# Nikhil-AI-Labs/image-super-resolution-2

Measured on AMD Instinct MI355X. Metric: output MPix/s at x4 SR (256->1024), higher is better.
Workload: dtype bf16 (bf16 MFMA operands, fp32 accumulate, fp32 activations in HBM); 1 GPU; FreqFusion x4 full 3-expert forward (HAT-L + DAT + NAFNet-SR + fusion stack), one 256x256 LR tile -> 1024x1024 per step per GPU (BASELINE configs[1]); seeded synthetic weights (172.3 M params), 1/f-noise tiles; tile=256, parallelism=tile-sharded x1, weights RCCL-broadcast once (0.0 ms), no per-tile collectives, launch=hipGraph replay, tiles_in_flight=2

## Files before the change

image-super-resolution-2_amd/csrc/token_linear.hip:

```cpp
#include "ff_common.h"


struct TokenLinParams {
  const float* x; float* out;
  const float* gamma; const float* beta;
  const __bf16* w;
  const float* bias;
  const float* res; const float* res2; const float* rs2;
  float* xn; int ldxn;
  float* stats; int st_lo, st_hi; float st_eps;
  const float* x2; int ldx2; const float* cm; const float* gw1t; const float* gb1; const float* gw2; float gb2;
  long long M;
  int ldx, ldo, ldr, ldr2, K, N, NT, act;
  float eps;
  int wpi;
};

#define TL_TR 36

#ifndef TL_GELU_SIG
#define TL_GELU_SIG 1
#endif
#define TL_KERNEL token_linear_kernel
#define TL_IMAGES 0
#define TL_OUT16 0
#include "token_linear_kernel.inc"
#undef TL_KERNEL
#undef TL_IMAGES
#define TL_KERNEL token_linear_images_kernel
#define TL_IMAGES 1
#include "token_linear_kernel.inc"
#undef TL_KERNEL
#undef TL_IMAGES
#undef TL_OUT16
#define TL_KERNEL token_linear_rows16_kernel
#define TL_IMAGES 0
#define TL_OUT16 1
#include "token_linear_kernel.inc"
#undef TL_KERNEL
#undef TL_IMAGES
#undef TL_OUT16


extern "C" int ff_token_linear(const float* x, int ldx, float* out, int ldo, long long M, int K, int kpad, int N, int n_tiles,
                               const float* gamma, const float* beta, float eps, const void* w_tiles,
                               const float* bias_padded, int act, const float* res, int ldr, const float* res2, int ldr2,
                               const float* res2_scale, float* xn_out, int ldxn, float* stats_out, int stat_lo, int stat_hi,
                               float stat_eps, int nterms, void* stream) {
  FF_CHECK_ARG(nterms == 1 || nterms == 3, "ff_token_linear: nterms must be 1 (plain bf16) or 3 (split bf16)");
  FF_CHECK_ARG(x && out && w_tiles, "ff_token_linear: null pointer");
  FF_CHECK_ARG(M > 0 && K > 0 && K <= 192 && K % 4 == 0 && N > 0 && n_tiles * 32 >= N, "ff_token_linear: needs K <= 192 (K %% 4 == 0), n_tiles*32 >= N");
  FF_CHECK_ARG(kpad == 64 || kpad == 128 || kpad == 192, "ff_token_linear: kpad must be 64, 128 or 192");
  FF_CHECK_ARG(kpad >= K, "ff_token_linear: kpad < K");
  FF_CHECK_ARG(ldx >= K && ldx % 4 == 0 && ldo >= N && (((uintptr_t)x) & 15) == 0, "ff_token_linear: x rows must be 16-byte aligned");
  FF_CHECK_ARG((gamma == nullptr) == (beta == nullptr), "ff_token_linear: gamma/beta come together");
  FF_CHECK_ARG((((uintptr_t)w_tiles) & 15) == 0 && (!gamma || ((((uintptr_t)gamma) & 15) == 0 && (((uintptr_t)beta) & 15) == 0)), "ff_token_linear: weights / gamma / beta must be 16-byte aligned");
  FF_CHECK_ARG(!res || ldr >= N, "ff_token_linear: ldr too small");
  FF_CHECK_ARG(!res2 || (ldr2 >= N && res2_scale), "ff_token_linear: res2 needs ldr2 >= N and a scale vector");
  FF_CHECK_ARG(!xn_out || (gamma && ldxn >= K && ldxn % 4 == 0 && (((uintptr_t)xn_out) & 15) == 0), "ff_token_linear: xn_out needs LayerNorm parameters and 16-byte aligned rows");
  TokenLinParams p;
  p.x = x; p.out = out; p.gamma = gamma; p.beta = beta; p.w = (const __bf16*)w_tiles; p.bias = bias_padded;
  p.res = res; p.res2 = res2; p.rs2 = res2_scale; p.xn = xn_out; p.ldxn = ldxn; p.M = M; p.ldx = ldx; p.ldo = ldo; p.ldr = ldr; p.ldr2 = ldr2;
  p.K = K; p.N = N; p.NT = n_tiles; p.act = act; p.eps = eps;
  FF_CHECK_ARG(!stats_out || (stat_lo >= 0 && stat_hi > stat_lo && stat_hi <= N && (((uintptr_t)stats_out) & 7) == 0), "ff_token_linear: bad statistics range");
  p.stats = stats_out; p.st_lo = stat_lo; p.st_hi = stat_hi; p.st_eps = stat_eps;
  p.x2 = nullptr; p.ldx2 = 0; p.cm = nullptr; p.gw1t = nullptr; p.gb1 = nullptr; p.gw2 = nullptr; p.gb2 = 0.f; p.wpi = 0;
  const bool vec4 = (N % 4 == 0) && (ldo % 4 == 0) && ((((uintptr_t)out) & 15) == 0) && (!res || (ldr % 4 == 0 && (((uintptr_t)res) & 15) == 0)) &&
           (!res2 || (ldr2 % 4 == 0 && (((uintptr_t)res2) & 15) == 0 && (((uintptr_t)res2_scale) & 15) == 0));
  const int ks = kpad / 16;
  const size_t lds = (size_t)2 * 2 * 32 * (2 * ks + 1) * 16 + (size_t)8 * 32 * TL_TR * 4 + (size_t)8 * 32 * FF_XS_ROW * 4 + (size_t)n_tiles * 32 * 4;
  FF_CHECK_ARG(lds <= 160 * 1024, "ff_token_linear: N too large for the LDS image");
  FF_CHECK_ARG(act == ACT_NONE || act == ACT_GELU, "ff_token_linear: act must be none or gelu");
  const long long nblk = (M + 255) / 256;
  FF_CHECK_ARG(nblk < (1LL << 31), "ff_token_linear: grid too large");
#define TL_LAUNCH(A, KSV, V4, NTM)                                                                                          \
  do {                                                                                                                      \
    static ff_device_once once;                                                                                             \
    if (!ff_raise_lds(once, "ff_token_linear", 160 * 1024, FF_LDS_SAY_ERR, &token_linear_kernel<A, KSV, V4, false, NTM>)) return FF_ERR_LAUNCH; \
    hipLaunchKernelGGL((token_linear_kernel<A, KSV, V4, false, NTM>), dim3((unsigned)nblk), dim3(512), lds, (hipStream_t)stream, p); \
  } while (0)
#define TL_LAUNCH_NT(A, KSV, V4) do { if (nterms == 3) TL_LAUNCH(A, KSV, V4, 3); else TL_LAUNCH(A, KSV, V4, 1); } while (0)
#define TL_LAUNCH_KS(A, V4) do { if (ks == 4) TL_LAUNCH_NT(A, 4, V4); else if (ks == 8) TL_LAUNCH_NT(A, 8, V4); else TL_LAUNCH_NT(A, 12, V4); } while (0)
  if (act == ACT_GELU) { if (vec4) TL_LAUNCH_KS(ACT_GELU, true); else TL_LAUNCH_KS(ACT_GELU, false); }
  else { if (vec4) TL_LAUNCH_KS(ACT_NONE, true); else TL_LAUNCH_KS(ACT_NONE, false); }
#undef TL_LAUNCH_KS
#undef TL_LAUNCH_NT
#undef TL_LAUNCH
  FF_LAUNCH_CHECK("ff_token_linear");
  return FF_OK;
}

extern "C" int ff_token_linear_rows16(const float* x, int ldx, void* out16, int ldo, long long M, int K, int kpad, int N, int n_tiles,
                                      const float* gamma, const float* beta, float eps, const void* w_tiles, const float* bias_padded,
                                      const float* col_scale, int act, const float* res, int ldr, const float* res2, int ldr2,
                                      const float* res2_scale, float* xn_out, int ldxn, float* stats_out, int stat_lo, int stat_hi,
                                      float stat_eps, int nterms, void* stream) {
  FF_CHECK_ARG(nterms == 1 && act == ACT_NONE && !res && !res2 && !res2_scale && !xn_out && !stats_out,
               "ff_token_linear_rows16: plain bf16 (nterms == 1), no activation, no res / res2 / xn_out / stats_out (got nterms=%d act=%d)", nterms, act);
  FF_CHECK_ARG(x && out16 && w_tiles && col_scale, "ff_token_linear_rows16: null pointer");
  FF_CHECK_ARG(M > 0 && K > 0 && K <= 192 && K % 4 == 0 && N > 0 && N % 4 == 0 && n_tiles * 32 >= N, "ff_token_linear_rows16: needs K <= 192, K and N multiples of 4, n_tiles*32 >= N");
  FF_CHECK_ARG(kpad == 64 || kpad == 128 || kpad == 192, "ff_token_linear_rows16: kpad must be 64, 128 or 192");
  FF_CHECK_ARG(kpad >= K, "ff_token_linear_rows16: kpad < K");
  FF_CHECK_ARG(ldx >= K && ldx % 4 == 0 && (((uintptr_t)x) & 15) == 0, "ff_token_linear_rows16: x rows must be 16-byte aligned");
  FF_CHECK_ARG(ldo >= N && ldo % 4 == 0 && (((uintptr_t)out16) & 7) == 0, "ff_token_linear_rows16: out rows must be 8-byte aligned (pitch in bf16 elements, a multiple of 4)");
  FF_CHECK_ARG((gamma == nullptr) == (beta == nullptr), "ff_token_linear_rows16: gamma/beta come together");
  FF_CHECK_ARG(((((uintptr_t)w_tiles) | ((uintptr_t)col_scale)) & 15) == 0 && (!gamma || ((((uintptr_t)gamma) & 15) == 0 && (((uintptr_t)beta) & 15) == 0)), "ff_token_linear_rows16: weights / col_scale / gamma / beta must be 16-byte aligned");
  TokenLinParams p;
  p.x = x; p.out = reinterpret_cast<float*>(out16); p.gamma = gamma; p.beta = beta; p.w = (const __bf16*)w_tiles; p.bias = bias_padded;
  p.res = nullptr; p.res2 = nullptr; p.rs2 = col_scale; p.xn = nullptr; p.ldxn = 0; p.M = M; p.ldx = ldx; p.ldo = ldo; p.ldr = 0; p.ldr2 = 0;
  p.K = K; p.N = N; p.NT = n_tiles; p.act = ACT_NONE; p.eps = eps;
  p.stats = nullptr; p.st_lo = 0; p.st_hi = 0; p.st_eps = 0.f;
  p.x2 = nullptr; p.ldx2 = 0; p.cm = nullptr; p.gw1t = nullptr; p.gb1 = nullptr; p.gw2 = nullptr; p.gb2 = 0.f; p.wpi = 0;
  const int ks = kpad / 16;
  const size_t lds = (size_t)2 * 2 * 32 * (2 * ks + 1) * 16 + (size_t)8 * 32 * TL_TR * 4 + (size_t)8 * 32 * FF_XS_ROW * 4 + (size_t)2 * n_tiles * 32 * 4;
  FF_CHECK_ARG(lds <= 160 * 1024, "ff_token_linear_rows16: N too large for the LDS image");
  const long long nblk = (M + 255) / 256;
  FF_CHECK_ARG(nblk < (1LL << 31), "ff_token_linear_rows16: grid too large");
#define TL_LAUNCH16(KSV)                                                                                                    \
  do {                                                                                                                      \
    static ff_device_once once;                                                                                             \
    if (!ff_raise_lds(once, "ff_token_linear_rows16", 160 * 1024, FF_LDS_SAY_ERR, &token_linear_rows16_kernel<ACT_NONE, KSV, true, false, 1>)) return FF_ERR_LAUNCH; \
    hipLaunchKernelGGL((token_linear_rows16_kernel<ACT_NONE, KSV, true, false, 1>), dim3((unsigned)nblk), dim3(512), lds, (hipStream_t)stream, p); \
  } while (0)
  if (ks == 4) TL_LAUNCH16(4); else if (ks == 8) TL_LAUNCH16(8); else TL_LAUNCH16(12);
#undef TL_LAUNCH16
  FF_LAUNCH_CHECK("ff_token_linear_rows16");
  return FF_OK;
}

static int token_linear_gated_launch(const char* who, const float* x, int ldx, const float* x2, int ldx2, const float* cm, int B, long long rows_per_image,
                                     const float* gw1t, const float* gb1, const float* gw2, float gb2, float* out, int ldo, long long M, int K, int N,
                                     int n_tiles, const void* w_tiles, const float* bias_padded, const float* res, int ldr, int nterms, void* stream) {
  FF_CHECK_ARG(nterms == 1 || nterms == 3, "%s: nterms must be 1 or 3", who);
  FF_CHECK_ARG(x && x2 && cm && gb1 && gw2 && out && w_tiles, "%s: null pointer", who);
  FF_CHECK_ARG(M > 0 && K > 0 && K <= 192 && K % 4 == 0 && N > 0 && N % 4 == 0 && n_tiles * 32 >= N, "%s: needs K <= 192, K and N multiples of 4", who);
  FF_CHECK_ARG(ldx >= K && ldx % 4 == 0 && ldx2 >= K && ldx2 % 4 == 0 && ldo >= N && ldo % 4 == 0 && (!res || (ldr >= N && ldr % 4 == 0)), "%s: rows must be 16-byte aligned", who);
  FF_CHECK_ARG(((((uintptr_t)x) | ((uintptr_t)x2) | ((uintptr_t)cm) | ((uintptr_t)out) | ((uintptr_t)w_tiles) | ((uintptr_t)res)) & 15) == 0, "%s: 16-byte alignment", who);
  const long long wpi = B ? rows_per_image / 256 : 0, nblk = B ? wpi : (M + 255) / 256;
  FF_CHECK_ARG(nblk < (1LL << 31), "%s: grid too large", who);
  TokenLinParams p{};
  p.x = x; p.out = out; p.w = (const __bf16*)w_tiles; p.bias = bias_padded; p.res = res; p.M = M; p.ldx = ldx; p.ldo = ldo; p.ldr = ldr;
  p.K = K; p.N = N; p.NT = n_tiles; p.act = ACT_NONE;
  p.x2 = x2; p.ldx2 = ldx2; p.cm = cm; p.gw1t = gw1t; p.gb1 = gb1; p.gw2 = gw2; p.gb2 = gb2; p.wpi = (int)wpi;
  const size_t lds = (size_t)2 * 2 * 32 * 25 * 16 + (size_t)8 * 32 * TL_TR * 4 + (size_t)8 * 32 * FF_XS_ROW * 4 + (size_t)n_tiles * 32 * 4;
  FF_CHECK_ARG(lds <= 160 * 1024, "%s: N too large for the LDS image", who);
  static ff_device_once once[2];
  if (!(!B ? ff_raise_lds(once[0], who, 160 * 1024, FF_LDS_SAY_ERR, &token_linear_kernel<ACT_NONE, 12, true, true, 3>, &token_linear_kernel<ACT_NONE, 12, true, true, 1>)
           : ff_raise_lds(once[1], who, 160 * 1024, FF_LDS_SAY_ERR, &token_linear_images_kernel<ACT_NONE, 12, true, true, 3>, &token_linear_images_kernel<ACT_NONE, 12, true, true, 1>)))
    return FF_ERR_LAUNCH;
  const dim3 grid((unsigned)nblk, B ? (unsigned)B : 1u);
  if (!B) {
    if (nterms == 3) hipLaunchKernelGGL((token_linear_kernel<ACT_NONE, 12, true, true, 3>), grid, dim3(512), lds, (hipStream_t)stream, p);
    else hipLaunchKernelGGL((token_linear_kernel<ACT_NONE, 12, true, true, 1>), grid, dim3(512), lds, (hipStream_t)stream, p);
  } else {
    if (nterms == 3) hipLaunchKernelGGL((token_linear_images_kernel<ACT_NONE, 12, true, true, 3>), grid, dim3(512), lds, (hipStream_t)stream, p);
    else hipLaunchKernelGGL((token_linear_images_kernel<ACT_NONE, 12, true, true, 1>), grid, dim3(512), lds, (hipStream_t)stream, p);
  }
  FF_LAUNCH_CHECK(who);
  return FF_OK;
}

extern "C" int ff_token_linear_gated(const float* x, int ldx, const float* x2, int ldx2, const float* cm, const float* gw1t,
                                     const float* gb1, const float* gw2, float gb2, float* out, int ldo, long long M, int K, int N,
                                     int n_tiles, const void* w_tiles, const float* bias_padded, const float* res, int ldr, int nterms,
                                     void* stream) {
  return token_linear_gated_launch("ff_token_linear_gated", x, ldx, x2, ldx2, cm, 0, 0, gw1t, gb1, gw2, gb2, out, ldo, M, K, N, n_tiles, w_tiles, bias_padded, res, ldr, nterms, stream);
}

extern "C" int ff_token_linear_gated_images(const float* x, int ldx, const float* x2, int ldx2, const float* cm, int B, long long rows_per_image,
                                            const float* gb1, const float* gw2, float gb2, float* out, int ldo, long long M, int K, int N,
                                            int n_tiles, const void* w_tiles, const float* bias_padded, const float* res, int ldr, int nterms,
                                            void* stream) {
  FF_CHECK_ARG(B > 0 && B <= 65535 && rows_per_image > 0 && rows_per_image % 256 == 0 && M == (long long)B * rows_per_image,
               "ff_token_linear_gated_images: rows_per_image must be a positive multiple of 256 and M == B * rows_per_image (1 <= B <= 65535; got B=%d rows_per_image=%lld M=%lld)",
               B, rows_per_image, M);
  return token_linear_gated_launch("ff_token_linear_gated_images", x, ldx, x2, ldx2, cm, B, rows_per_image, nullptr, gb1, gw2, gb2, out, ldo, M, K, N, n_tiles, w_tiles, bias_padded, res, ldr, nterms, stream);
}
```

image-super-resolution-2_amd/csrc/token_linear_kernel.inc:

```
template <int ACT, int TL_KS, bool VEC4, bool GATED = false, int NTERMS = 3>
__global__ __launch_bounds__(512) void TL_KERNEL(TokenLinParams p) {
  constexpr int TL_SLOTS = 2 * TL_KS + 1, TL_ROWB = TL_SLOTS * 16, TL_PL = 32 * TL_SLOTS, TL_PIECES = 2 * TL_PL / 64;
  constexpr int TL_TILE_ELEMS = 32 * 16 * TL_KS, KPAD = 16 * TL_KS;
  extern __shared__ __attribute__((aligned(16))) unsigned char smem[];
  constexpr int WB = TL_PL * 16;
  constexpr int BUFB = 2 * WB;
  const int tid = threadIdx.x, lane = tid & 63, wid = tid >> 6;
  const int l31 = lane & 31, hh = lane >> 5;
  float* tr = reinterpret_cast<float*>(smem + 2 * BUFB) + wid * (32 * TL_TR);
  float* xs = reinterpret_cast<float*>(smem + 2 * BUFB + 8 * 32 * TL_TR * 4) + wid * (32 * FF_XS_ROW);
  float* Bs = reinterpret_cast<float*>(smem + 2 * BUFB + 8 * 32 * TL_TR * 4 + 8 * 32 * FF_XS_ROW * 4);
#if TL_IMAGES
  const long long tok0 = ((long long)blockIdx.y * p.wpi + blockIdx.x) * 256 + wid * 32;
  const float* cmrow = p.cm + (long long)blockIdx.y * p.K;
#else
  const long long tok0 = (long long)blockIdx.x * 256 + wid * 32;
  const float* cmrow = p.cm;
#endif
  const long long tok = tok0 + l31;
  const bool tvalid = tok < p.M;

  int off[4];
#pragma unroll
  for (int i = 0; i < 4; ++i) {
    int s = (wid + 8 * i) * 64 + lane;
    if (s >= 2 * TL_PL) s = 2 * TL_PL - 1;
    const int plane = s / TL_PL, t = s - plane * TL_PL, row = t / TL_SLOTS;
    int q = t - row * TL_SLOTS;
    if (q > 2 * TL_KS - 1) q = 2 * TL_KS - 1;
    off[i] = plane * TL_TILE_ELEMS + row * KPAD + q * 8;
  }
  auto dma = [&](int nt, int buf) {
    const __bf16* rec = p.w + (long long)nt * (2 * TL_TILE_ELEMS);
#pragma unroll
    for (int i = 0; i < 4; ++i)
      if (wid + 8 * i < TL_PIECES)
        __builtin_amdgcn_global_load_lds((const __attribute__((address_space(1))) void*)(rec + off[i]),
                                         (__attribute__((address_space(3))) void*)(smem + buf * BUFB + (wid + 8 * i) * 1024), 16, 0, 0);
  };
  dma(0, 0);
  for (int i = tid; i < p.NT * 32; i += 512) Bs[i] = p.bias ? p.bias[i] : 0.f;
#if TL_OUT16
  float* Ss = Bs + p.NT * 32;
  for (int i = tid; i < p.NT * 32; i += 512) Ss[i] = p.rs2[i];
#endif

  bf16x8 xh[TL_KS], xl[TL_KS];
  if constexpr (GATED) {
    dma(p.NT, 1);
    float sm;
    {
      bf16x8 th[TL_KS], tl[TL_KS];
      {
        float v[TL_KS][8];
        ff_wave_rows_to_frags<TL_KS / 4>(p.x, p.ldx, tok0, p.M, p.K, xs, lane, v);
#pragma unroll
        for (int st = 0; st < TL_KS; ++st)
#pragma unroll
          for (int j = 0; j < 8; ++j) {
            const __bf16 h = (__bf16)v[st][j];
            th[st][j] = h;
            if (NTERMS == 3) tl[st][j] = (__bf16)(v[st][j] - (float)h);
          }
      }
      asm volatile("s_waitcnt vmcnt(0)" ::: "memory");
      __syncthreads();
      const unsigned char* ap = smem + BUFB + l31 * TL_ROWB + 16 * hh;
      f32x16 ga;
#pragma unroll
      for (int r = 0; r < 16; ++r) ga[r] = p.gb1[(r & 3) + 8 * (r >> 2) + 4 * hh];
#define TL_XH th
#define TL_XL tl
#define TL_ACC ga
#include "token_linear_tile_mfma.inc"
#undef TL_XH
#undef TL_XL
#undef TL_ACC
      float sacc = 0.f;
#pragma unroll
      for (int r = 0; r < 16; ++r) sacc += p.gw2[(r & 3) + 8 * (r >> 2) + 4 * hh] * ff_gelu_fast(ga[r]);
      sacc += __shfl_xor(sacc, 32);
      sm = 1.0f / (1.0f + expf(-(sacc + p.gb2)));
    }
    asm volatile("" ::: "memory");
    const int rr = lane >> 4, cq = (lane & 15) * 4;
#pragma unroll
    for (int pass = 0; pass < TL_KS / 4; ++pass) {
      asm volatile("" ::: "memory");
      f32x4 tS[8], tO[8];
#pragma unroll
      for (int j = 0; j < 8; ++j) {
        const int r = 4 * j + rr, c = 64 * pass + cq;
        const bool ok = tok0 + r < p.M && c < p.K;
        const f32x4 u = *reinterpret_cast<const f32x4*>(p.x + (ok ? (tok0 + r) * p.ldx + c : 0));
        const f32x4 w2 = *reinterpret_cast<const f32x4*>(p.x2 + (ok ? (tok0 + r) * p.ldx2 + c : 0));
        tS[j] = ok ? u : (f32x4){0.f, 0.f, 0.f, 0.f};
        tO[j] = ok ? w2 : (f32x4){0.f, 0.f, 0.f, 0.f};
      }
#pragma unroll
      for (int j = 0; j < 8; ++j) *reinterpret_cast<f32x4*>(xs + (4 * j + rr) * FF_XS_ROW + cq) = tS[j];
      f32x4 sa[4], sb[4];
#pragma unroll
      for (int s4 = 0; s4 < 4; ++s4) {
        sa[s4] = *reinterpret_cast<const f32x4*>(xs + l31 * FF_XS_ROW + 16 * s4 + 8 * hh);
        sb[s4] = *reinterpret_cast<const f32x4*>(xs + l31 * FF_XS_ROW + 16 * s4 + 8 * hh + 4);
      }
#pragma unroll
      for (int j = 0; j < 8; ++j) *reinterpret_cast<f32x4*>(xs + (4 * j + rr) * FF_XS_ROW + cq) = tO[j];
#pragma unroll
      for (int s4 = 0; s4 < 4; ++s4) {
        const int st = 4 * pass + s4, k0 = 16 * st + 8 * hh;
        const f32x4 oa = *reinterpret_cast<const f32x4*>(xs + l31 * FF_XS_ROW + 16 * s4 + 8 * hh);
        const f32x4 ob = *reinterpret_cast<const f32x4*>(xs + l31 * FF_XS_ROW + 16 * s4 + 8 * hh + 4);
        const int ka = k0 < p.K ? k0 : 0, kb = k0 + 4 < p.K ? k0 + 4 : 0;
        const f32x4 ca = *reinterpret_cast<const f32x4*>(cmrow + ka), cb = *reinterpret_cast<const f32x4*>(cmrow + kb);
        bf16x8 nh, nl;
#pragma unroll
        for (int j = 0; j < 8; ++j) {
          const float o = j < 4 ? oa[j & 3] : ob[j & 3], cmv = j < 4 ? ca[j & 3] : cb[j & 3];
          const float sv = j < 4 ? sa[s4][j & 3] : sb[s4][j & 3];
          const float f = (k0 + j < p.K) ? sv * cmv + o * sm : 0.f;
          const __bf16 h = (__bf16)f;
          nh[j] = h;
          if (NTERMS == 3) nl[j] = (__bf16)(f - (float)h);
        }
        xh[st] = nh;
        if (NTERMS == 3) {
          xl[st] = nl;
          asm volatile("" : "+v"(xh[st]), "+v"(xl[st]) : : "memory");
        } else {
          asm volatile("" : "+v"(xh[st]) : : "memory");
        }
      }
    }
  } else
  {
    float v[TL_KS][8];
    ff_wave_rows_to_frags<TL_KS / 4>(p.x, p.ldx, tok0, p.M, p.K, xs, lane, v);
    float mean = 0.f, rstd = 1.f;
    if (p.gamma) {
      float s = 0.f;
#pragma unroll
      for (int st = 0; st < TL_KS; ++st)
#pragma unroll
        for (int j = 0; j < 8; ++j) s += v[st][j];
      s += __shfl_xor(s, 32);
      mean = s / (float)p.K;
      float qv = 0.f;
#pragma unroll
      for (int st = 0; st < TL_KS; ++st)
#pragma unroll
        for (int j = 0; j < 8; ++j) {
          const float d = (16 * st + 8 * hh + j < p.K) ? v[st][j] - mean : 0.f;
          qv += d * d;
        }
      qv += __shfl_xor(qv, 32);
      rstd = 1.0f / sqrtf(qv / (float)p.K + p.eps);
    }
#define LN_OPT_KS TL_KS
#define LN_OPT_TOK tok
#include "frag_ln_opt_step.inc"
#undef LN_OPT_KS
#undef LN_OPT_TOK
  }

  float ssum = 0.f, ssq = 0.f;
  asm volatile("s_waitcnt vmcnt(0)" ::: "memory");
  for (int nt = 0; nt < p.NT; ++nt) {
    const int buf = nt & 1;
    asm volatile("s_waitcnt lgkmcnt(0)" ::: "memory");
    __builtin_amdgcn_s_barrier();
    if (nt + 1 < p.NT) dma(nt + 1, buf ^ 1);
    const int col = nt * 32 + l31;
    const bool cok = col < p.N;
    const int cc = cok ? col : 0;
    const int tq = lane >> 3, c4 = nt * 32 + 4 * (lane & 7);
    const bool c4ok = c4 < p.N;
    float rv[16];
    f32x4 rq[4];
    if (VEC4 && !TL_OUT16) {
#pragma unroll
      for (int i = 0; i < 4; ++i) {
        const long long tk = tok0 + tq + 8 * i;
        const bool ok = c4ok && tk < p.M;
        f32x4 r0 = {0.f, 0.f, 0.f, 0.f};
        if (p.res) { const f32x4 u = *reinterpret_cast<const f32x4*>(p.res + (ok ? tk * p.ldr + c4 : 0)); r0 = ok ? u : r0; }
        if (p.res2) {
          const f32x4 u = *reinterpret_cast<const f32x4*>(p.res2 + (ok ? tk * p.ldr2 + c4 : 0));
          const f32x4 sc = *reinterpret_cast<const f32x4*>(p.rs2 + (c4ok ? c4 : 0));
          if (ok) r0 += u * sc;
        }
        rq[i] = r0;
      }
    } else if (!VEC4) {
#pragma unroll
      for (int i = 0; i < 16; ++i) {
        const long long tk = tok0 + 2 * i + hh;
        const long long tqq = tk < p.M ? tk : 0;
        float r0 = p.res ? p.res[tqq * p.ldr + cc] : 0.f;
        if (p.res2) r0 += p.res2[tqq * p.ldr2 + cc] * p.rs2[cc];
        rv[i] = r0;
      }
    }
    const unsigned char* ap = smem + buf * BUFB + l31 * TL_ROWB + 16 * hh;
    f32x16 acc;
    {
      const int nb = nt * 32 + 4 * hh;
#pragma unroll
      for (int r = 0; r < 16; ++r) acc[r] = Bs[nb + (r & 3) + 8 * (r >> 2)];
    }
#define TL_XH xh
#define TL_XL xl
#define TL_ACC acc
#include "token_linear_tile_mfma.inc"
#undef TL_XH
#undef TL_XL
#undef TL_ACC
#pragma unroll
    for (int g = 0; g < 4; ++g) {
      f32x4 v4;
      if (ACT == ACT_GELU && NTERMS == 1 && TL_GELU_SIG) {
        const f32x2 ga = ff_gelu_sig2((f32x2){acc[4 * g], acc[4 * g + 1]}), gb = ff_gelu_sig2((f32x2){acc[4 * g + 2], acc[4 * g + 3]});
        v4 = (f32x4){ga[0], ga[1], gb[0], gb[1]};
      } else {
#pragma unroll
        for (int e = 0; e < 4; ++e) v4[e] = ff_act_c<ACT, true>(acc[4 * g + e]);
      }
      *reinterpret_cast<f32x4*>(tr + l31 * TL_TR + 8 * g + 4 * hh) = v4;
      if (p.stats) {
        const int c0 = nt * 32 + 8 * g + 4 * hh;
#pragma unroll
        for (int e = 0; e < 4; ++e)
          if (c0 + e >= p.st_lo && c0 + e < p.st_hi) { ssum += v4[e]; ssq += v4[e] * v4[e]; }
      }
    }
    asm volatile("s_waitcnt vmcnt(0)" ::: "memory");
#if TL_OUT16
    {
      const f32x4 cs = *reinterpret_cast<const f32x4*>(Ss + nt * 32 + 4 * (lane & 7));
      bf16x4 ov[4];
#pragma unroll
      for (int i = 0; i < 4; ++i) {
        const f32x4 t4 = *reinterpret_cast<const f32x4*>(tr + (tq + 8 * i) * TL_TR + 4 * (lane & 7)) * cs;
        ov[i] = (bf16x4){(__bf16)t4[0], (__bf16)t4[1], (__bf16)t4[2], (__bf16)t4[3]};
      }
      if (c4ok) {
        __bf16* op = reinterpret_cast<__bf16*>(p.out) + (tok0 + tq) * p.ldo + c4;
        if (tok0 + 32 <= p.M) {
#pragma unroll
          for (int i = 0; i < 4; ++i) *reinterpret_cast<bf16x4*>(op + (long long)(8 * i) * p.ldo) = ov[i];
        } else {
#pragma unroll
          for (int i = 0; i < 4; ++i)
            if (tok0 + tq + 8 * i < p.M) *reinterpret_cast<bf16x4*>(op + (long long)(8 * i) * p.ldo) = ov[i];
        }
      }
    }
#else
    if (VEC4) {
      f32x4 ov[4];
#pragma unroll
      for (int i = 0; i < 4; ++i) ov[i] = *reinterpret_cast<const f32x4*>(tr + (tq + 8 * i) * TL_TR + 4 * (lane & 7)) + rq[i];
      if (c4ok) {
        float* op = p.out + (tok0 + tq) * p.ldo + c4;
        if (tok0 + 32 <= p.M) {
#pragma unroll
          for (int i = 0; i < 4; ++i) *reinterpret_cast<f32x4*>(op + (long long)(8 * i) * p.ldo) = ov[i];
        } else {
#pragma unroll
          for (int i = 0; i < 4; ++i)
            if (tok0 + tq + 8 * i < p.M) *reinterpret_cast<f32x4*>(op + (long long)(8 * i) * p.ldo) = ov[i];
        }
      }
    } else {
      float ov[16];
#pragma unroll
      for (int i = 0; i < 16; ++i) ov[i] = tr[(2 * i + hh) * TL_TR + l31] + rv[i];
      if (cok) {
        float* op = p.out + (tok0 + hh) * p.ldo + col;
        if (tok0 + 32 <= p.M) {
#pragma unroll
          for (int i = 0; i < 16; ++i) op[(long long)(2 * i) * p.ldo] = ov[i];
        } else {
#pragma unroll
          for (int i = 0; i < 16; ++i)
            if (tok0 + 2 * i + hh < p.M) op[(long long)(2 * i) * p.ldo] = ov[i];
        }
      }
    }
#endif
  }
  if (p.stats) {
    ssum += __shfl_xor(ssum, 32);
    ssq += __shfl_xor(ssq, 32);
    const float n = (float)(p.st_hi - p.st_lo);
    const float mean = ssum / n;
    const float var = fmaxf(ssq / n - mean * mean, 0.f);
    if (hh == 0 && tvalid) *reinterpret_cast<float2*>(p.stats + 2 * tok) = make_float2(mean, 1.0f / sqrtf(var + p.st_eps));
  }
}
```

Measured before the change: 28.33 output MPix/s.

## Shrink token-linear LDS footprint and block size to fit two blocks per CU

```diff
diff --git a/image-super-resolution-2_amd/csrc/token_linear.hip b/image-super-resolution-2_amd/csrc/token_linear.hip
--- a/image-super-resolution-2_amd/csrc/token_linear.hip
+++ b/image-super-resolution-2_amd/csrc/token_linear.hip
@@ -17,6 +17,26 @@
 };
 
 #define TL_TR 36
+
+template <int KS, int NTERMS>
+struct TokenLinRing {
+  static constexpr int PLANES = NTERMS == 1 ? 1 : 2;
+  static constexpr int PLANE_BYTES = 32 * (2 * KS + 1) * 16;
+  static constexpr int PIECES = (PLANES * PLANE_BYTES + 1023) / 1024;
+  static constexpr int SLOT_BYTES = PIECES * 1024;
+  static constexpr int NW = (NTERMS == 1 && KS < 12) ? 4 : 8;
+  static constexpr size_t LDS_MAX = (size_t)NW * 20 * 1024;
+};
+struct TokenLinShape { int nw; size_t lds, lds_max; };
+template <int KS, int NTERMS>
+static TokenLinShape token_linear_shape_of(int n_tiles, bool col_scale) {
+  using R = TokenLinRing<KS, NTERMS>;
+  return {R::NW, 2 * (size_t)R::SLOT_BYTES + (size_t)R::NW * 32 * FF_XS_ROW * 4 + (size_t)(col_scale ? 2 : 1) * n_tiles * 32 * 4, R::LDS_MAX};
+}
+static TokenLinShape token_linear_shape(int ks, int nterms, int n_tiles, bool col_scale) {
+  if (nterms == 1) return ks == 4 ? token_linear_shape_of<4, 1>(n_tiles, col_scale) : ks == 8 ? token_linear_shape_of<8, 1>(n_tiles, col_scale) : token_linear_shape_of<12, 1>(n_tiles, col_scale);
+  return ks == 4 ? token_linear_shape_of<4, 3>(n_tiles, col_scale) : ks == 8 ? token_linear_shape_of<8, 3>(n_tiles, col_scale) : token_linear_shape_of<12, 3>(n_tiles, col_scale);
+}
 
 #ifndef TL_GELU_SIG
 #define TL_GELU_SIG 1
@@ -68,16 +88,19 @@
   const bool vec4 = (N % 4 == 0) && (ldo % 4 == 0) && ((((uintptr_t)out) & 15) == 0) && (!res || (ldr % 4 == 0 && (((uintptr_t)res) & 15) == 0)) &&
            (!res2 || (ldr2 % 4 == 0 && (((uintptr_t)res2) & 15) == 0 && (((uintptr_t)res2_scale) & 15) == 0));
   const int ks = kpad / 16;
-  const size_t lds = (size_t)2 * 2 * 32 * (2 * ks + 1) * 16 + (size_t)8 * 32 * TL_TR * 4 + (size_t)8 * 32 * FF_XS_ROW * 4 + (size_t)n_tiles * 32 * 4;
-  FF_CHECK_ARG(lds <= 160 * 1024, "ff_token_linear: N too large for the LDS image");
+  const TokenLinShape sh = token_linear_shape(ks, nterms, n_tiles, false);
+  const size_t lds = sh.lds;
+  const int nw = sh.nw;
+  FF_CHECK_ARG(lds <= sh.lds_max, "ff_token_linear: N too large for the LDS image");
   FF_CHECK_ARG(act == ACT_NONE || act == ACT_GELU, "ff_token_linear: act must be none or gelu");
-  const long long nblk = (M + 255) / 256;
+  const long long nblk = (M + 32 * nw - 1) / (32 * nw);
   FF_CHECK_ARG(nblk < (1LL << 31), "ff_token_linear: grid too large");
 #define TL_LAUNCH(A, KSV, V4, NTM)                                                                                          \
   do {                                                                                                                      \
+    using R = TokenLinRing<KSV, NTM>;                                                                                       \
     static ff_device_once once;                                                                                             \
-    if (!ff_raise_lds(once, "ff_token_linear", 160 * 1024, FF_LDS_SAY_ERR, &token_linear_kernel<A, KSV, V4, false, NTM>)) return FF_ERR_LAUNCH; \
-    hipLaunchKernelGGL((token_linear_kernel<A, KSV, V4, false, NTM>), dim3((unsigned)nblk), dim3(512), lds, (hipStream_t)stream, p); \
+    if (!ff_raise_lds(once, "ff_token_linear", R::LDS_MAX, FF_LDS_SAY_ERR, &token_linear_kernel<A, KSV, V4, false, NTM, R::NW>)) return FF_ERR_LAUNCH; \
+    hipLaunchKernelGGL((token_linear_kernel<A, KSV, V4, false, NTM, R::NW>), dim3((unsigned)nblk), dim3(R::NW * 64), lds, (hipStream_t)stream, p); \
   } while (0)
 #define TL_LAUNCH_NT(A, KSV, V4) do { if (nterms == 3) TL_LAUNCH(A, KSV, V4, 3); else TL_LAUNCH(A, KSV, V4, 1); } while (0)
 #define TL_LAUNCH_KS(A, V4) do { if (ks == 4) TL_LAUNCH_NT(A, 4, V4); else if (ks == 8) TL_LAUNCH_NT(A, 8, V4); else TL_LAUNCH_NT(A, 12, V4); } while (0)
@@ -112,15 +135,17 @@
   p.stats = nullptr; p.st_lo = 0; p.st_hi = 0; p.st_eps = 0.f;
   p.x2 = nullptr; p.ldx2 = 0; p.cm = nullptr; p.gw1t = nullptr; p.gb1 = nullptr; p.gw2 = nullptr; p.gb2 = 0.f; p.wpi = 0;
   const int ks = kpad / 16;
-  const size_t lds = (size_t)2 * 2 * 32 * (2 * ks + 1) * 16 + (size_t)8 * 32 * TL_TR * 4 + (size_t)8 * 32 * FF_XS_ROW * 4 + (size_t)2 * n_tiles * 32 * 4;
-  FF_CHECK_ARG(lds <= 160 * 1024, "ff_token_linear_rows16: N too large for the LDS image");
-  const long long nblk = (M + 255) / 256;
+  const TokenLinShape sh = token_linear_shape(ks, 1, n_tiles, true);
+  const size_t lds = sh.lds;
+  FF_CHECK_ARG(lds <= sh.lds_max, "ff_token_linear_rows16: N too large for the LDS image");
+  const long long nblk = (M + 32 * sh.nw - 1) / (32 * sh.nw);
   FF_CHECK_ARG(nblk < (1LL << 31), "ff_token_linear_rows16: grid too large");
 #define TL_LAUNCH16(KSV)                                                                                                    \
   do {                                                                                                                      \
+    using R = TokenLinRing<KSV, 1>;                                                                                         \
     static ff_device_once once;                                                                                             \
-    if (!ff_raise_lds(once, "ff_token_linear_rows16", 160 * 1024, FF_LDS_SAY_ERR, &token_linear_rows16_kernel<ACT_NONE, KSV, true, false, 1>)) return FF_ERR_LAUNCH; \
-    hipLaunchKernelGGL((token_linear_rows16_kernel<ACT_NONE, KSV, true, false, 1>), dim3((unsigned)nblk), dim3(512), lds, (hipStream_t)stream, p); \
+    if (!ff_raise_lds(once, "ff_token_linear_rows16", R::LDS_MAX, FF_LDS_SAY_ERR, &token_linear_rows16_kernel<ACT_NONE, KSV, true, false, 1, R::NW>)) return FF_ERR_LAUNCH; \
+    hipLaunchKernelGGL((token_linear_rows16_kernel<ACT_NONE, KSV, true, false, 1, R::NW>), dim3((unsigned)nblk), dim3(R::NW * 64), lds, (hipStream_t)stream, p); \
   } while (0)
   if (ks == 4) TL_LAUNCH16(4); else if (ks == 8) TL_LAUNCH16(8); else TL_LAUNCH16(12);
 #undef TL_LAUNCH16
@@ -136,25 +161,31 @@
   FF_CHECK_ARG(M > 0 && K > 0 && K <= 192 && K % 4 == 0 && N > 0 && N % 4 == 0 && n_tiles * 32 >= N, "%s: needs K <= 192, K and N multiples of 4", who);
   FF_CHECK_ARG(ldx >= K && ldx % 4 == 0 && ldx2 >= K && ldx2 % 4 == 0 && ldo >= N && ldo % 4 == 0 && (!res || (ldr >= N && ldr % 4 == 0)), "%s: rows must be 16-byte aligned", who);
   FF_CHECK_ARG(((((uintptr_t)x) | ((uintptr_t)x2) | ((uintptr_t)cm) | ((uintptr_t)out) | ((uintptr_t)w_tiles) | ((uintptr_t)res)) & 15) == 0, "%s: 16-byte alignment", who);
-  const long long wpi = B ? rows_per_image / 256 : 0, nblk = B ? wpi : (M + 255) / 256;
+  const TokenLinShape sh = token_linear_shape(12, nterms, n_tiles, false);
+  const int nw = sh.nw;
+  const long long wpi = B ? rows_per_image / (32 * nw) : 0, nblk = B ? wpi : (M + 32 * nw - 1) / (32 * nw);
   FF_CHECK_ARG(nblk < (1LL << 31), "%s: grid too large", who);
   TokenLinParams p{};
   p.x = x; p.out = out; p.w = (const __bf16*)w_tiles; p.bias = bias_padded; p.res = res; p.M = M; p.ldx = ldx; p.ldo = ldo; p.ldr = ldr;
   p.K = K; p.N = N; p.NT = n_tiles; p.act = ACT_NONE;
   p.x2 = x2; p.ldx2 = ldx2; p.cm = cm; p.gw1t = gw1t; p.gb1 = gb1; p.gw2 = gw2; p.gb2 = gb2; p.wpi = (int)wpi;
-  const size_t lds = (size_t)2 * 2 * 32 * 25 * 16 + (size_t)8 * 32 * TL_TR * 4 + (size_t)8 * 32 * FF_XS_ROW * 4 + (size_t)n_tiles * 32 * 4;
-  FF_CHECK_ARG(lds <= 160 * 1024, "%s: N too large for the LDS image", who);
-  static ff_device_once once[2];
-  if (!(!B ? ff_raise_lds(once[0], who, 160 * 1024, FF_LDS_SAY_ERR, &token_linear_kernel<ACT_NONE, 12, true, true, 3>, &token_linear_kernel<ACT_NONE, 12, true, true, 1>)
-           : ff_raise_lds(once[1], who, 160 * 1024, FF_LDS_SAY_ERR, &token_linear_images_kernel<ACT_NONE, 12, true, true, 3>, &token_linear_images_kernel<ACT_NONE, 12, true, true, 1>)))
+  using R3 = TokenLinRing<12, 3>;
+  using R1 = TokenLinRing<12, 1>;
+  const size_t lds = sh.lds;
+  FF_CHECK_ARG(lds <= sh.lds_max, "%s: N too large for the LDS image", who);
+  static ff_device_once once[4];
+  if (!(!B ? (nterms == 3 ? ff_raise_lds(once[0], who, R3::LDS_MAX, FF_LDS_SAY_ERR, &token_linear_kernel<ACT_NONE, 12, true, true, 3, R3::NW>)
+                          : ff_raise_lds(once[1], who, R1::LDS_MAX, FF_LDS_SAY_ERR, &token_linear_kernel<ACT_NONE, 12, true, true, 1, R1::NW>))
+           : (nterms == 3 ? ff_raise_lds(once[2], who, R3::LDS_MAX, FF_LDS_SAY_ERR, &token_linear_images_kernel<ACT_NONE, 12, true, true, 3, R3::NW>)
+                          : ff_raise_lds(once[3], who, R1::LDS_MAX, FF_LDS_SAY_ERR, &token_linear_images_kernel<ACT_NONE, 12, true, true, 1, R1::NW>))))
     return FF_ERR_LAUNCH;
   const dim3 grid((unsigned)nblk, B ? (unsigned)B : 1u);
   if (!B) {
-    if (nterms == 3) hipLaunchKernelGGL((token_linear_kernel<ACT_NONE, 12, true, true, 3>), grid, dim3(512), lds, (hipStream_t)stream, p);
-    else hipLaunchKernelGGL((token_linear_kernel<ACT_NONE, 12, true, true, 1>), grid, dim3(512), lds, (hipStream_t)stream, p);
+    if (nterms == 3) hipLaunchKernelGGL((token_linear_kernel<ACT_NONE, 12, true, true, 3, R3::NW>), grid, dim3(R3::NW * 64), lds, (hipStream_t)stream, p);
+    else hipLaunchKernelGGL((token_linear_kernel<ACT_NONE, 12, true, true, 1, R1::NW>), grid, dim3(R1::NW * 64), lds, (hipStream_t)stream, p);
   } else {
-    if (nterms == 3) hipLaunchKernelGGL((token_linear_images_kernel<ACT_NONE, 12, true, true, 3>), grid, dim3(512), lds, (hipStream_t)stream, p);
-    else hipLaunchKernelGGL((token_linear_images_kernel<ACT_NONE, 12, true, true, 1>), grid, dim3(512), lds, (hipStream_t)stream, p);
+    if (nterms == 3) hipLaunchKernelGGL((token_linear_images_kernel<ACT_NONE, 12, true, true, 3, R3::NW>), grid, dim3(R3::NW * 64), lds, (hipStream_t)stream, p);
+    else hipLaunchKernelGGL((token_linear_images_kernel<ACT_NONE, 12, true, true, 1, R1::NW>), grid, dim3(R1::NW * 64), lds, (hipStream_t)stream, p);
   }
   FF_LAUNCH_CHECK(who);
   return FF_OK;
diff --git a/image-super-resolution-2_amd/csrc/token_linear_kernel.inc b/image-super-resolution-2_amd/csrc/token_linear_kernel.inc
--- a/image-super-resolution-2_amd/csrc/token_linear_kernel.inc
+++ b/image-super-resolution-2_amd/csrc/token_linear_kernel.inc
@@ -1,30 +1,35 @@
-template <int ACT, int TL_KS, bool VEC4, bool GATED = false, int NTERMS = 3>
-__global__ __launch_bounds__(512) void TL_KERNEL(TokenLinParams p) {
-  constexpr int TL_SLOTS = 2 * TL_KS + 1, TL_ROWB = TL_SLOTS * 16, TL_PL = 32 * TL_SLOTS, TL_PIECES = 2 * TL_PL / 64;
+template <int ACT, int TL_KS, bool VEC4, bool GATED = false, int NTERMS = 3, int NW = 8>
+__global__ __launch_bounds__(NW * 64, 2) void TL_KERNEL(TokenLinParams p) {
+  constexpr int TL_SLOTS = 2 * TL_KS + 1, TL_ROWB = TL_SLOTS * 16, TL_PL = 32 * TL_SLOTS;
+  constexpr int TL_PLANES = TokenLinRing<TL_KS, NTERMS>::PLANES;
+  constexpr int TL_PIECES = TokenLinRing<TL_KS, NTERMS>::PIECES;
+  constexpr int TL_NI = (TL_PIECES + NW - 1) / NW;
   constexpr int TL_TILE_ELEMS = 32 * 16 * TL_KS, KPAD = 16 * TL_KS;
   extern __shared__ __attribute__((aligned(16))) unsigned char smem[];
   constexpr int WB = TL_PL * 16;
-  constexpr int BUFB = 2 * WB;
+  constexpr int BUFB = TokenLinRing<TL_KS, NTERMS>::SLOT_BYTES;
+  static_assert(BUFB >= TL_PIECES * 1024 && BUFB >= TL_PLANES * WB && TL_PIECES * 64 >= TL_PLANES * TL_PL, "a tile's DMA pieces cover its planes and stay inside its ring slot");
+  static_assert(TL_TR <= FF_XS_ROW, "the transpose patch lives inside the wave's staging patch");
   const int tid = threadIdx.x, lane = tid & 63, wid = tid >> 6;
   const int l31 = lane & 31, hh = lane >> 5;
-  float* tr = reinterpret_cast<float*>(smem + 2 * BUFB) + wid * (32 * TL_TR);
-  float* xs = reinterpret_cast<float*>(smem + 2 * BUFB + 8 * 32 * TL_TR * 4) + wid * (32 * FF_XS_ROW);
-  float* Bs = reinterpret_cast<float*>(smem + 2 * BUFB + 8 * 32 * TL_TR * 4 + 8 * 32 * FF_XS_ROW * 4);
+  float* xs = reinterpret_cast<float*>(smem + 2 * BUFB) + wid * (32 * FF_XS_ROW);
+  float* tr = xs;
+  float* Bs = reinterpret_cast<float*>(smem + 2 * BUFB + NW * 32 * FF_XS_ROW * 4);
 #if TL_IMAGES
-  const long long tok0 = ((long long)blockIdx.y * p.wpi + blockIdx.x) * 256 + wid * 32;
+  const long long tok0 = ((long long)blockIdx.y * p.wpi + blockIdx.x) * (32 * NW) + wid * 32;
   const float* cmrow = p.cm + (long long)blockIdx.y * p.K;
 #else
-  const long long tok0 = (long long)blockIdx.x * 256 + wid * 32;
+  const long long tok0 = (long long)blockIdx.x * (32 * NW) + wid * 32;
   const float* cmrow = p.cm;
 #endif
   const long long tok = tok0 + l31;
   const bool tvalid = tok < p.M;
 
-  int off[4];
-#pragma unroll
-  for (int i = 0; i < 4; ++i) {
-    int s = (wid + 8 * i) * 64 + lane;
-    if (s >= 2 * TL_PL) s = 2 * TL_PL - 1;
+  int off[TL_NI];
+#pragma unroll
+  for (int i = 0; i < TL_NI; ++i) {
+    int s = (wid + NW * i) * 64 + lane;
+    if (s >= TL_PLANES * TL_PL) s = TL_PLANES * TL_PL - 1;
     const int plane = s / TL_PL, t = s - plane * TL_PL, row = t / TL_SLOTS;
     int q = t - row * TL_SLOTS;
     if (q > 2 * TL_KS - 1) q = 2 * TL_KS - 1;
@@ -33,16 +38,16 @@
   auto dma = [&](int nt, int buf) {
     const __bf16* rec = p.w + (long long)nt * (2 * TL_TILE_ELEMS);
 #pragma unroll
-    for (int i = 0; i < 4; ++i)
-      if (wid + 8 * i < TL_PIECES)
+    for (int i = 0; i < TL_NI; ++i)
+      if (wid + NW * i < TL_PIECES)
         __builtin_amdgcn_global_load_lds((const __attribute__((address_space(1))) void*)(rec + off[i]),
-                                         (__attribute__((address_space(3))) void*)(smem + buf * BUFB + (wid + 8 * i) * 1024), 16, 0, 0);
+                                         (__attribute__((address_space(3))) void*)(smem + buf * BUFB + (wid + NW * i) * 1024), 16, 0, 0);
   };
   dma(0, 0);
-  for (int i = tid; i < p.NT * 32; i += 512) Bs[i] = p.bias ? p.bias[i] : 0.f;
+  for (int i = tid; i < p.NT * 32; i += NW * 64) Bs[i] = p.bias ? p.bias[i] : 0.f;
 #if TL_OUT16
   float* Ss = Bs + p.NT * 32;
-  for (int i = tid; i < p.NT * 32; i += 512) Ss[i] = p.rs2[i];
+  for (int i = tid; i < p.NT * 32; i += NW * 64) Ss[i] = p.rs2[i];
 #endif
 
   bf16x8 xh[TL_KS], xl[TL_KS];
```

Result: no change. 28.56 output MPix/s (median of 6 runs) (+0.8%).
